# lucasgattas/ComfyUI-Egregora-Audio-Super-Resolution

Measured on AMD Instinct MI355X. Metric: audio-sec/sec (xRT) FlashSR 48kHz + Fat-Llama 800-iter at 1/2/4/8 MI355X, higher is better.
Workload: dtype f32(f16x2); 1 GPU; chain60: per GPU 60 s stereo 48 kHz; FlashSR (5.12 s chunks, hop 4.62 s, student_ldm 1-step + VAE + sr_vocoder, declared architecture, synthetic weights, chunk-sharded with one all-gather, WOLA) then Fat-Llama max_iterations=800 thr=0.6 normalize on autoscale off, threshold reading of the HEADLINE value: 'default' (SPEC.md section 3 default = absolute level on int16-scale samples, hard threshold, ; arch=gfx950:sramecc+:xnack-, chunks=13, rows_per_pass=32

## Files before the change

### comfyui-egregora-audio-super-resolution_amd/csrc/egr_nn_ops.hip

```cpp
#include <math.h>
#include <string.h>

#include <vector>

#include <stdlib.h>
#include <string.h>

#include "egr_common.h"
#include "egr_rowmax.h"
#include "egr_stft_tables.h"
#include "egr_plan.h"

namespace egr {

__global__ __launch_bounds__(256) void k_gn_stats(const float* __restrict__ x, int HW, int C, int G,
                                                   double* __restrict__ stats , int slab) {
    const int b = blockIdx.y;
    const int p0 = blockIdx.x * slab;
    const int p1 = min(HW, p0 + slab);
    const int cpg = C / G;
    const float* xb = x + (size_t)b * HW * C;
    for (int c = threadIdx.x; c < C; c += blockDim.x) {
        float s = 0.f, ss = 0.f;
        for (int p = p0; p < p1; ++p) {
// ... 261 lines not shown
        if (r0 + k < R && c0 + tx < Cc) t[k][tx] = x[off + (size_t)(r0 + k) * Cc + c0 + tx];
    __syncthreads();
    for (int k = ty; k < 32; k += 8)
        if (c0 + k < Cc && r0 + tx < R) y[off + (size_t)(c0 + k) * R + r0 + tx] = t[tx][k];
}

__global__ __launch_bounds__(256) void k_snake_aa(const float* __restrict__ x, const float* __restrict__ alpha,
                                                   const float* __restrict__ beta, const float* __restrict__ filt,
                                                   float* __restrict__ y, int L, int C, int K) {
    __shared__ float f[32];
    if (threadIdx.x < K) f[threadIdx.x] = filt[threadIdx.x];
    __syncthreads();
    const int b = blockIdx.z;
    const int c = blockIdx.x * 64 + (threadIdx.x & 63);
    const int l = blockIdx.y * 4 + (threadIdx.x >> 6);
    if (c >= C || l >= L) return;
    const float* xb = x + (size_t)b * L * C + c;
    const float a = __expf(alpha[c]), ib = 1.0f / (__expf(beta[c]) + 1e-9f);
    const int pad = K / 2 - 1;
    const int pl = pad * 2 + (K - 2) / 2;
    const int L2 = 2 * L;
    float acc = 0.f;
    for (int k = 0; k < K; ++k) {
        int i = 2 * l + k - (K / 2 - 1);
        i = i < 0 ? 0 : (i > L2 - 1 ? L2 - 1 : i);
        const int t = i + pl;
        int n_lo = (t - (K - 1) + 1) >> 1;
        if (2 * n_lo < t - (K - 1)) ++n_lo;
        const int n_hi = t >> 1;
        float u = 0.f;
        for (int n = n_lo; n <= n_hi; ++n) {
            int src = n - pad;
            src = src < 0 ? 0 : (src > L - 1 ? L - 1 : src);
            u += xb[(size_t)src * C] * f[t - 2 * n];
        }
        u *= 2.0f;
        const float sn = __sinf(u * a);
        acc += f[k] * (u + ib * sn * sn);
    }
    y[(size_t)b * L * C + (size_t)l * C + c] = acc;
}


template <int CB, int TL>
__global__ __launch_bounds__(256) void k_snake_aa_tiled(const float* __restrict__ x, const float* __restrict__ alpha,
                                                        const float* __restrict__ beta, const float* __restrict__ filt,
                                                        float* __restrict__ y, int L, int C) {
    constexpr int PL = 256 / CB, K = 12, XT = TL + 10, ST = 2 * TL + 10;
    __shared__ float xs[XT][CB];
    __shared__ float ss[ST][CB];
    __shared__ float f[K];
    if (threadIdx.x < K) f[threadIdx.x] = filt[threadIdx.x];
    const int c = threadIdx.x % CB, pl = threadIdx.x / CB;
    const int c0 = blockIdx.x * CB, l0 = blockIdx.y * TL, b = blockIdx.z;
    const float* xb = x + (size_t)b * L * C + c0 + c;
    for (int p = pl; p < XT; p += PL) {
        int src = l0 - 5 + p;
        src = src < 0 ? 0 : (src > L - 1 ? L - 1 : src);
        xs[p][c] = xb[(size_t)src * C];
    }
    const float a = __expf(alpha[c0 + c]), ib = 1.0f / (__expf(beta[c0 + c]) + 1e-9f);
    __syncthreads();
    const int L2 = 2 * L;
    for (int q = pl; q < ST; q += PL) {
        int i = 2 * l0 - 5 + q;
        i = i < 0 ? 0 : (i > L2 - 1 ? L2 - 1 : i);
        const int t = i + 15;
        const int n_hi = t >> 1;
        float u = 0.f;
#pragma unroll
        for (int j = 0; j < 6; ++j) {
            const int n = n_hi - j;
            int p = n - l0;
            p = p < 0 ? 0 : (p > XT - 1 ? XT - 1 : p);
            u += xs[p][c] * f[t - 2 * n];
        }
        u *= 2.0f;
        const float sn = __sinf(u * a);
        ss[q][c] = u + ib * sn * sn;
    }
    __syncthreads();
    float* yb = y + (size_t)b * L * C + c0 + c;
    for (int j = pl; j < TL; j += PL) {
        const int l = l0 + j;
        if (l >= L) break;
        float acc = 0.f;
#pragma unroll
        for (int k = 0; k < K; ++k) acc += f[k] * ss[2 * j + k][c];
        yb[(size_t)l * C] = acc;
    }
}

template <int J>
__global__ __launch_bounds__(256) void k_snake_aa_reg(const float* __restrict__ x, const float* __restrict__ alpha,
                                                      const float* __restrict__ beta, const float* __restrict__ filt,
                                                      float* __restrict__ y, int L, int C, int nruns,
                                                      unsigned* __restrict__ row_amax) {
    const int b = blockIdx.y;
    const long long per_row = (long long)nruns * C;
    float ymax = 0.f;
    for (long long gid = (long long)blockIdx.x * 256 + threadIdx.x; gid < per_row; gid += (long long)gridDim.x * 256) {
    const int c = (int)(gid % C);
    const int run = (int)(gid / C);
    const int l0 = run * J;
    float f[12];
#pragma unroll
    for (int k = 0; k < 12; ++k) f[k] = filt[k];
    const float a = __expf(alpha[c]), ib = 1.0f / (__expf(beta[c]) + 1e-9f);
    const float* xb = x + (size_t)b * L * C + c;
    float* yb = y + (size_t)b * L * C + c;
    const int L2 = 2 * L;
    float xw[J + 10];
#pragma unroll
    for (int i = 0; i < J + 10; ++i) {
        int src = l0 - 5 + i;
        src = src < 0 ? 0 : (src > L - 1 ? L - 1 : src);
        xw[i] = xb[(size_t)src * C];
    }
    float sv[2 * J + 10];
#pragma unroll
    for (int q = 0; q < 2 * J + 10; ++q) {
        float u = 0.f;
#pragma unroll
        for (int j = 0; j < 6; ++j) u += xw[5 + (q >> 1) - j] * f[(q & 1) + 2 * j];
        u *= 2.0f;
        const float sn = __sinf(u * a);
        sv[q] = u + ib * sn * sn;
    }
    const int i0 = 2 * l0 - 5;
    if (i0 < 0 || i0 + 2 * J + 9 > L2 - 1) {
        float s_first = 0.f, s_last = 0.f;
#pragma unroll
        for (int q = 0; q < 2 * J + 10; ++q) {
            if (i0 + q == 0) s_first = sv[q];
            if (i0 + q == L2 - 1) s_last = sv[q];
        }
#pragma unroll
        for (int q = 0; q < 2 * J + 10; ++q) {
            if (i0 + q < 0) sv[q] = s_first;
            if (i0 + q > L2 - 1) sv[q] = s_last;
        }
    }
#pragma unroll
    for (int jj = 0; jj < J; ++jj) {
        float acc = 0.f;
#pragma unroll
        for (int k = 0; k < 12; ++k) acc += f[k] * sv[2 * jj + k];
        if (l0 + jj < L) { yb[(size_t)(l0 + jj) * C] = acc; ymax = fmaxf(ymax, fabsf(acc)); }
    }
    }
    if (row_amax) row_amax_commit_wg(row_amax + (size_t)b * EGR_ROW_AMAX_STRIDE, ymax);
}

__global__ __launch_bounds__(256) void k_col2im1d(const float* __restrict__ Y, const float* __restrict__ bias,
                                                   const float* __restrict__ add, float* __restrict__ out, int Lin,
                                                   int Lout, int Co, int K, int r, int pad, long long n) {
    for (long long i = (long long)blockIdx.x * blockDim.x + threadIdx.x; i < n;
         i += (long long)gridDim.x * blockDim.x) {
        const int co = (int)(i % Co);
        const long long t = i / Co;
        const int o = (int)(t % Lout);
        const long long b = t / Lout;
        float v = bias ? bias[co] : 0.f;
        if (add) v += add[i];
        const int q = o + pad;
        for (int k = q % r; k < K; k += r) {
            const int ii = (q - k) / r;
            if (q - k >= 0 && ii < Lin) v += Y[(((size_t)b * Lin + ii) * K + k) * Co + co];
        }
        out[i] = v;
    }
}

__global__ __launch_bounds__(256) void k_stft_frames(const float* __restrict__ x, int L, int n_fft, int hop, int rpad,
                                                      int T, int t_valid, int ldm, const float* __restrict__ window,
                                                      FftDesc fd, const cplx* __restrict__ tw,
                                                      const cplx* __restrict__ wsplit, float* __restrict__ mag) {
    extern __shared__ __attribute__((aligned(16))) char smem[];
    const int Mh = n_fft / 2;
    cplx* cur = (cplx*)smem;
    cplx* alt = cur + Mh;
    const int t = blockIdx.x, b = blockIdx.y;
    float* o = mag + ((size_t)b * T + t) * ldm;
    if (t >= t_valid) {
        for (int k = threadIdx.x; k < ldm; k += blockDim.x) o[k] = 0.f;
        return;
    }
    const float* xb = x + (size_t)b * L;
    const int s0 = t * hop - rpad;
    for (int e = threadIdx.x; e < Mh; e += blockDim.x) {
        float v[2];
#pragma unroll
        for (int h = 0; h < 2; ++h) {
            int i = s0 + 2 * e + h;
            if (i < 0) i = -i;
            if (i > L - 1) i = 2 * (L - 1) - i;
            i = i < 0 ? 0 : (i > L - 1 ? L - 1 : i);
            v[h] = xb[i] * window[2 * e + h];
        }
        cur[e] = make_float2(v[0], v[1]);
    }
    __syncthreads();
    lds_fft<false>(cur, alt, fd, tw, 1, 0, 1, Mh, false);
    for (int k = threadIdx.x; k < ldm; k += blockDim.x) {
        float r = 0.f;
        if (k <= Mh) {
            const cplx Za = cur[k == Mh ? 0 : k];
            const cplx Zb = cur[(k == 0 || k == Mh) ? 0 : Mh - k];
            const cplx E = make_float2(0.5f * (Za.x + Zb.x), 0.5f * (Za.y - Zb.y));
            const cplx O = make_float2(0.5f * (Za.y + Zb.y), -0.5f * (Za.x - Zb.x));
            const cplx X = cadd(E, cmul(wsplit[k], O));
            r = sqrtf(X.x * X.x + X.y * X.y);
        }
        o[k] = r;
    }
}

__device__ __forceinline__ void philox_round(unsigned& c0, unsigned& c1, unsigned& c2, unsigned& c3, unsigned k0,
                                             unsigned k1) {
    const unsigned long long p0 = (unsigned long long)0xD2511F53u * c0;
    const unsigned long long p1 = (unsigned long long)0xCD9E8D57u * c2;
    const unsigned n0 = (unsigned)(p1 >> 32) ^ c1 ^ k0, n1 = (unsigned)p1;
    const unsigned n2 = (unsigned)(p0 >> 32) ^ c3 ^ k1, n3 = (unsigned)p0;
    c0 = n0; c1 = n1; c2 = n2; c3 = n3;
}

__global__ __launch_bounds__(256) void k_randn(float* __restrict__ out, long long per_row, int rows,
                                                unsigned long long seed, const long long* __restrict__ row_ids, long long id_base) {
    const long long quads = (per_row + 3) / 4;
    const long long n = quads * rows;
    for (long long i = (long long)blockIdx.x * blockDim.x + threadIdx.x; i < n;
         i += (long long)gridDim.x * blockDim.x) {
        const int r = (int)(i / quads);
        const long long q = i - (long long)r * quads;
        const unsigned long long rid = row_ids ? (unsigned long long)row_ids[r] : (unsigned long long)(id_base + r);
        unsigned c0 = (unsigned)q, c1 = (unsigned)(q >> 32), c2 = (unsigned)rid, c3 = (unsigned)(rid >> 32);
        unsigned k0 = (unsigned)seed, k1 = (unsigned)(seed >> 32);
#pragma unroll
        for (int it = 0; it < 10; ++it) {
            philox_round(c0, c1, c2, c3, k0, k1);
            k0 += 0x9E3779B9u;
            k1 += 0xBB67AE85u;
        }
        const float u0 = ((float)c0 + 0.5f) * 2.3283064365386963e-10f, u1 = ((float)c1 + 0.5f) * 2.3283064365386963e-10f;
        const float u2 = ((float)c2 + 0.5f) * 2.3283064365386963e-10f, u3 = ((float)c3 + 0.5f) * 2.3283064365386963e-10f;
        const float r0 = sqrtf(-2.0f * logf(u0)), r1 = sqrtf(-2.0f * logf(u2));
        float z[4];
        z[0] = r0 * cosf(6.283185307179586f * u1);
        z[1] = r0 * sinf(6.283185307179586f * u1);
        z[2] = r1 * cosf(6.283185307179586f * u3);
        z[3] = r1 * sinf(6.283185307179586f * u3);
        float* o = out + (size_t)r * per_row + q * 4;
        for (int j = 0; j < 4; ++j)
            if (q * 4 + j < per_row) o[j] = z[j];
    }
}

__global__ __launch_bounds__(256) void k_wino_in(const float* __restrict__ x, int B, int H, int W, int C, int TH, int TW,
                                                  const float* __restrict__ gsc, const float* __restrict__ gsh, int gsilu,
                                                  float* __restrict__ V) {
    const int C4 = C >> 2;
    const long long P = (long long)B * TH * TW, total = P * C4;
    for (long long i = (long long)blockIdx.x * blockDim.x + threadIdx.x; i < total; i += (long long)gridDim.x * blockDim.x) {
        const int c4 = (int)(i % C4);
        const long long t = i / C4;
        const int tx = (int)(t % TW), ty = (int)((t / TW) % TH), b = (int)(t / ((long long)TW * TH));
        float4 d[4][4];
        float4 sc = make_float4(1.f, 1.f, 1.f, 1.f), sh = make_float4(0.f, 0.f, 0.f, 0.f);
        if (gsc) {
            sc = *(const float4*)(gsc + (size_t)b * C + 4 * c4);
            sh = *(const float4*)(gsh + (size_t)b * C + 4 * c4);
        }
#pragma unroll
        for (int r = 0; r < 4; ++r) {
            const int iy = 2 * ty - 1 + r;
#pragma unroll
            for (int q = 0; q < 4; ++q) {
                const int ix = 2 * tx - 1 + q;
                const bool ok = (unsigned)iy < (unsigned)H && (unsigned)ix < (unsigned)W;
                const size_t off = ok ? (((size_t)b * H + iy) * W + ix) * C + 4 * c4 : (size_t)(4 * c4);
                float4 v = *(const float4*)(x + off);
                if (gsc) {
                    v = make_float4(v.x * sc.x + sh.x, v.y * sc.y + sh.y, v.z * sc.z + sh.z, v.w * sc.w + sh.w);
                    if (gsilu) {
                        v.x = v.x / (1.f + __expf(-v.x)); v.y = v.y / (1.f + __expf(-v.y));
                        v.z = v.z / (1.f + __expf(-v.z)); v.w = v.w / (1.f + __expf(-v.w));
                    }
                }
                d[r][q] = ok ? v : make_float4(0.f, 0.f, 0.f, 0.f);
            }
        }
#define F4OP(a, op, b) make_float4(a.x op b.x, a.y op b.y, a.z op b.z, a.w op b.w)
        float4 r_[4][4];
#pragma unroll
        for (int q = 0; q < 4; ++q) {
            r_[0][q] = F4OP(d[0][q], -, d[2][q]);
            r_[1][q] = F4OP(d[1][q], +, d[2][q]);
            r_[2][q] = F4OP(d[2][q], -, d[1][q]);
            r_[3][q] = F4OP(d[1][q], -, d[3][q]);
        }
        float* o = V + (size_t)t * C + 4 * c4;
        const size_t zs = (size_t)P * C;
#pragma unroll
        for (int r = 0; r < 4; ++r) {
            *(float4*)(o + (size_t)(4 * r + 0) * zs) = F4OP(r_[r][0], -, r_[r][2]);
            *(float4*)(o + (size_t)(4 * r + 1) * zs) = F4OP(r_[r][1], +, r_[r][2]);
// ... 213 lines not shown
extern "C" int egr_groupnorm_coeff_from_stats(const double* stats, const float* gamma, const float* beta, int B, int HW, int C,
                                              int G, float eps, float* scale, float* shift, void* stream) {
    EGR_CHECK(stats && gamma && beta && scale && shift && B >= 1 && HW >= 1 && C >= 1 && G >= 1 && C % G == 0, EGR_ERR_ARG,
              "bad argument");
    hipLaunchKernelGGL(k_gn_coeff, dim3((B * C + 255) / 256), dim3(256), 0, (hipStream_t)stream, stats, gamma, beta, scale, shift,
                       B, C, G, (double)HW * (C / G), eps);
    EGR_HIP(hipGetLastError());
    return EGR_OK;
}

extern "C" int egr_gn_operand_bound(const float* scale, const float* shift, int B, int C, const float* x_row_amax, float* bound, void* stream) {
    EGR_CHECK(scale && shift && x_row_amax && bound && B >= 1 && C >= 1, EGR_ERR_ARG, "bad argument");
    hipLaunchKernelGGL(k_gn_bound, dim3(B), dim3(256), 0, (hipStream_t)stream, scale, shift, C, x_row_amax, bound);
    EGR_HIP(hipGetLastError());
    return EGR_OK;
}

extern "C" size_t egr_groupnorm_workspace_bytes(int B, int C, int G) {
    return sizeof(double) * (size_t)B * G * 2 + sizeof(float) * 2 * (size_t)B * C + 64;
}

extern "C" int egr_layernorm_rows_ra(const float* x, const float* gamma, const float* beta, float* y, int64_t rows, int C,
                                     float eps, int batch_rows, float* row_amax, void* stream) {
    EGR_CHECK(x && gamma && beta && y && rows >= 1 && C >= 1 && batch_rows >= 1 && batch_rows <= 65535 && rows % batch_rows == 0, EGR_ERR_ARG,
              "bad argument");
    const long long per_b = rows / batch_rows;
    long long nx = (per_b + 3) / 4, cap = std::max<long long>(1, 16384 / batch_rows);
    if (nx > cap) nx = cap;
    hipLaunchKernelGGL(k_layernorm, dim3((unsigned)nx, (unsigned)batch_rows), dim3(256), 0, (hipStream_t)stream, x, gamma, beta, y,
                       (int)per_b, C, eps, (unsigned*)row_amax);
    EGR_HIP(hipGetLastError());
    return EGR_OK;
}

extern "C" int egr_layernorm_rows(const float* x, const float* gamma, const float* beta, float* y, int64_t rows, int C,
                                  float eps, void* stream) {
    int g = 1;
    for (int c : {64, 32, 16, 8, 4, 2}) if (rows % c == 0) { g = c; break; }
    return egr_layernorm_rows_ra(x, gamma, beta, y, rows, C, eps, g, nullptr, stream);
}

extern "C" int egr_softmax_rows(float* x, int64_t rows, int cols, void* stream) {
    EGR_CHECK(x && rows >= 1 && cols >= 1, EGR_ERR_ARG, "bad argument");
    const dim3 grid((unsigned)rows), blk(256);
    if (cols <= 1024) hipLaunchKernelGGL(k_softmax_reg<4>, grid, blk, 0, (hipStream_t)stream, x, cols);
    else if (cols <= 2048) hipLaunchKernelGGL(k_softmax_reg<8>, grid, blk, 0, (hipStream_t)stream, x, cols);
    else if (cols <= 4096) hipLaunchKernelGGL(k_softmax_reg<16>, grid, blk, 0, (hipStream_t)stream, x, cols);
    else hipLaunchKernelGGL(k_softmax, grid, blk, 0, (hipStream_t)stream, x, cols);
    EGR_HIP(hipGetLastError());
    return EGR_OK;
}

extern "C" int egr_eltwise_ra(const float* a, const float* b, float* y, int64_t n, int op, float s0, float s1, int batch_rows,
                              float* row_amax, void* stream) {
    EGR_CHECK(a && y && n >= 0 && op >= 0 && op <= 5 && batch_rows >= 1 && batch_rows <= 65535 && n % batch_rows == 0, EGR_ERR_ARG, "bad argument");
    EGR_CHECK(b || (op != EW_ADD && op != EW_AXPBY && op != EW_ADD_SCALE), EGR_ERR_ARG, "binary op needs b");
    if (n == 0) return EGR_OK;
    const long long per = n / batch_rows;
    hipLaunchKernelGGL(k_eltwise, dim3(row_grid_x(per, batch_rows, 8192, 4), (unsigned)batch_rows), dim3(256), 0, (hipStream_t)stream, a, b, y, per,
                       op, s0, s1, (unsigned*)row_amax);
    EGR_HIP(hipGetLastError());
    return EGR_OK;
}

extern "C" int egr_eltwise(const float* a, const float* b, float* y, int64_t n, int op, float s0, float s1, void* stream) {
    int g = 1;
    for (int c : {64, 32, 16, 8, 4, 2}) if (n % c == 0) { g = c; break; }
    return egr_eltwise_ra(a, b, y, n, op, s0, s1, g, nullptr, stream);
}

extern "C" int egr_geglu_ra(const float* u, float* y, int64_t rows, int D, int batch_rows, float* row_amax, void* stream) {
    EGR_CHECK(u && y && rows >= 1 && D >= 1 && batch_rows >= 1 && batch_rows <= 65535 && rows % batch_rows == 0, EGR_ERR_ARG, "bad argument");
    const long long per = rows / batch_rows;
    hipLaunchKernelGGL(k_geglu, dim3(row_grid_x(per * D, batch_rows, 8192, 4), (unsigned)batch_rows), dim3(256), 0, (hipStream_t)stream, u, y, per, D,
                       (unsigned*)row_amax);
    EGR_HIP(hipGetLastError());
    return EGR_OK;
}

extern "C" int egr_geglu(const float* u, float* y, int64_t rows, int D, void* stream) {
    int g = 1;
    for (int c : {64, 32, 16, 8, 4, 2}) if (rows % c == 0) { g = c; break; }
    return egr_geglu_ra(u, y, rows, D, g, nullptr, stream);
}

extern "C" int egr_tap_gather(const float* P, const float* bias, float* y, int B, int H, int W, int KH, int KW, int Cout, int pad_t,
                              int pad_l, void* stream) {
    EGR_CHECK(P && y && B >= 1 && H >= 1 && W >= 1 && KH >= 1 && KW >= 1 && Cout >= 1, EGR_ERR_ARG, "bad argument");
    hipLaunchKernelGGL(k_tap_gather, dim3(grid1d((long long)B * H * W * Cout)), dim3(256), 0, (hipStream_t)stream, P, bias, y, B, H, W,
                       KH, KW, Cout, pad_t, pad_l);
    EGR_HIP(hipGetLastError());
    return EGR_OK;
}

extern "C" int egr_conv_cin1(const float* x, const float* w_packed, const float* bias, float* y, int B, int H, int W, int Cout, int KH,
                             int KW, int pad_t, int pad_l, void* stream) {
    EGR_CHECK(x && w_packed && y && B >= 1 && H >= 1 && W >= 1 && Cout >= 4 && Cout % 4 == 0 && 256 % (Cout / 4) == 0, EGR_ERR_ARG,
              "bad argument (Cout / 4 must divide 256)");
    EGR_CHECK((KH == 3 && KW == 3) || (KH == 1 && KW == 1), EGR_ERR_UNSUPPORTED, "one-input-channel conv: 3x3 or 1x1 only");
    EGR_CHECK((long long)B * H * W < (1ll << 31), EGR_ERR_ARG, "image too large for 32-bit pixel indices");
    EGR_CHECK((((uintptr_t)y) & 15) == 0 && (!bias || (((uintptr_t)bias) & 15) == 0), EGR_ERR_ARG, "y / bias need 16-byte alignment");
    const int ppi = 256 / (Cout / 4);
    long long nb = ((long long)B * H * W + ppi - 1) / ppi;
    if (nb > 8192) nb = 8192;
    if (KH == 3) hipLaunchKernelGGL((k_conv_cin1<9>), dim3((unsigned)nb), dim3(256), 0, (hipStream_t)stream, x, w_packed, bias, y, B, H, W,
                                    Cout, KW, pad_t, pad_l);
    else hipLaunchKernelGGL((k_conv_cin1<1>), dim3((unsigned)nb), dim3(256), 0, (hipStream_t)stream, x, w_packed, bias, y, B, H, W, Cout,
                            KW, pad_t, pad_l);
    EGR_HIP(hipGetLastError());
    return EGR_OK;
}

extern "C" int egr_concat_channels_ra(const float* a, const float* b, float* y, int64_t M, int C1, int C2, int batch_rows, float* row_amax,
                                      void* stream) {
    EGR_CHECK(a && b && y && M >= 1 && C1 >= 1 && C2 >= 1 && batch_rows >= 1 && batch_rows <= 65535 && M % batch_rows == 0, EGR_ERR_ARG, "bad argument");
    const long long per = M / batch_rows;
    hipLaunchKernelGGL(k_concat, dim3(row_grid_x(per * (C1 + C2), batch_rows, 8192, 4), (unsigned)batch_rows), dim3(256), 0, (hipStream_t)stream, a, b, y,
                       per, C1, C2, (unsigned*)row_amax);
    EGR_HIP(hipGetLastError());
    return EGR_OK;
}

extern "C" int egr_concat_channels(const float* a, const float* b, float* y, int64_t M, int C1, int C2, void* stream) {
    int g = 1;
    for (int c : {64, 32, 16, 8, 4, 2}) if (M % c == 0) { g = c; break; }
    return egr_concat_channels_ra(a, b, y, M, C1, C2, g, nullptr, stream);
}

extern "C" int egr_transpose_batched(const float* x, float* y, int batch, int R, int Cc, void* stream) {
    EGR_CHECK(x && y && batch >= 1 && batch <= 65535 && R >= 1 && Cc >= 1, EGR_ERR_ARG, "bad argument");
    hipLaunchKernelGGL(k_transpose, dim3((Cc + 31) / 32, (R + 31) / 32, batch), dim3(256), 0, (hipStream_t)stream, x, y, R,
                       Cc);
    EGR_HIP(hipGetLastError());
    return EGR_OK;
}

extern "C" int egr_snake_aa_ra(const float* x, const float* alpha, const float* beta, const float* filt, float* y, int B,
                               int L, int C, int K, float* row_amax, void* stream);
extern "C" int egr_snake_aa(const float* x, const float* alpha, const float* beta, const float* filt, float* y, int B,
                            int L, int C, int K, void* stream) {
    return egr_snake_aa_ra(x, alpha, beta, filt, y, B, L, C, K, nullptr, stream);
}

extern "C" int egr_snake_aa_ra(const float* x, const float* alpha, const float* beta, const float* filt, float* y, int B,
                               int L, int C, int K, float* row_amax, void* stream) {
    EGR_CHECK(x && alpha && beta && filt && y && B >= 1 && B <= 65535 && L >= 1 && C >= 1 && K >= 2 && K <= 32 && K % 2 == 0,
              EGR_ERR_ARG, "bad argument");
    hipStream_t st = (hipStream_t)stream;
    static const bool tiled = getenv("EGR_SNAKE") && !strcmp(getenv("EGR_SNAKE"), "tiled");
    if (K == 12 && !tiled) {
        constexpr int J = 16;
        const int nruns = (L + J - 1) / J;
        static const int max_wg = getenv("EGR_SNAKE_WG") ? atoi(getenv("EGR_SNAKE_WG")) : 8192;
        hipLaunchKernelGGL((k_snake_aa_reg<J>), dim3(row_grid_x((long long)nruns * C, B, max_wg), (unsigned)B), dim3(256), 0, st, x, alpha, beta, filt, y, L, C,
                           nruns, (unsigned*)row_amax);
        row_amax = nullptr;
    } else if (K == 12 && C % 64 == 0)
        hipLaunchKernelGGL((k_snake_aa_tiled<64, 32>), dim3(C / 64, (L + 31) / 32, B), dim3(256), 0, st, x, alpha, beta, filt, y, L, C);
    else if (K == 12 && C % 32 == 0)
        hipLaunchKernelGGL((k_snake_aa_tiled<32, 64>), dim3(C / 32, (L + 63) / 64, B), dim3(256), 0, st, x, alpha, beta, filt, y, L, C);
    else if (K == 12 && C % 16 == 0)
        hipLaunchKernelGGL((k_snake_aa_tiled<16, 128>), dim3(C / 16, (L + 127) / 128, B), dim3(256), 0, st, x, alpha, beta, filt, y, L, C);
    else
        hipLaunchKernelGGL(k_snake_aa, dim3((C + 63) / 64, (L + 3) / 4, B), dim3(256), 0, st, x, alpha, beta, filt, y, L, C, K);
    EGR_HIP(hipGetLastError());
    if (row_amax) return egr_absmax_rows(y, B, (int64_t)L * C, 1, 0, row_amax, stream);
    return EGR_OK;
}

extern "C" int egr_col2im_convtr1d(const float* Y, const float* bias, const float* add, float* out, int B, int Lin,
                                   int Lout, int Co, int K, int r, int pad, void* stream) {
    EGR_CHECK(Y && out && B >= 1 && Lin >= 1 && Lout >= 1 && Co >= 1 && K >= 1 && r >= 1 && pad >= 0, EGR_ERR_ARG,
              "bad argument");
    const long long n = (long long)B * Lout * Co;
    hipLaunchKernelGGL(k_col2im1d, dim3(grid1d(n)), dim3(256), 0, (hipStream_t)stream, Y, bias, add, out, Lin, Lout, Co, K,
                       r, pad, n);
    EGR_HIP(hipGetLastError());
    return EGR_OK;
}

extern "C" int egr_stft_frames(const float* x, int B, int L, int n_fft, int hop, int rpad, int T, int t_valid, int ldm,
                               const float* window, float* mag, void* stream) {
    EGR_CHECK(x && window && mag && B >= 1 && B <= 65535 && L >= 2 && hop >= 1 && T >= 1 && t_valid >= 0 && t_valid <= T,
              EGR_ERR_ARG, "bad argument");
    EGR_CHECK(n_fft >= 4 && n_fft % 2 == 0 && n_fft <= 8192 && ldm >= n_fft / 2 + 1 && rpad < L, EGR_ERR_UNSUPPORTED,
              "bad STFT geometry");
    StftTables t;
    int rc = stft_tables(n_fft, &t);
    if (rc) return rc;
    const size_t lds = (size_t)2 * (n_fft / 2) * sizeof(float2);
    hipLaunchKernelGGL(k_stft_frames, dim3(T, B), dim3(256), lds, (hipStream_t)stream, x, L, n_fft, hop, rpad, T, t_valid,
                       ldm, window, t.fd, t.tw, t.wsplit, mag);
    EGR_HIP(hipGetLastError());
    return EGR_OK;
}

extern "C" int egr_randn_base(float* out, int64_t per_row, int rows, uint64_t seed, const int64_t* row_ids, int64_t id_base, void* stream) {
    EGR_CHECK(out && per_row >= 1 && rows >= 1, EGR_ERR_ARG, "bad argument");
    const long long n = ((per_row + 3) / 4) * rows;
    hipLaunchKernelGGL(k_randn, dim3(grid1d(n)), dim3(256), 0, (hipStream_t)stream, out, (long long)per_row, rows,
                       (unsigned long long)seed, (const long long*)row_ids, (long long)id_base);
    EGR_HIP(hipGetLastError());
    return EGR_OK;
}

extern "C" int egr_randn(float* out, int64_t per_row, int rows, uint64_t seed, const int64_t* row_ids, void* stream) {
    return egr_randn_base(out, per_row, rows, seed, row_ids, 0, stream);
}

extern "C" int egr_lowpass_gain(const float* mag, int B, int T, int ldm, int nb, float pct, float sr, int order,
                                float ripple_db, int64_t nbins, int* cut_out, float* gain, void* stream) {
    EGR_CHECK(mag && cut_out && gain && B >= 1 && B <= 65535 && T >= 1 && nb >= 2 && nb <= ldm && nbins >= 2 && order >= 1,
              EGR_ERR_ARG, "bad argument");
    hipStream_t st = (hipStream_t)stream;
    hipLaunchKernelGGL(k_cutoff_bin, dim3(B), dim3(256), nb * sizeof(float), st, mag, T, ldm, nb, pct, cut_out);
    const float eps2 = powf(10.0f, ripple_db / 10.0f) - 1.0f;
    hipLaunchKernelGGL(k_cheby_gain, dim3(grid1d(nbins), B), dim3(256), 0, st, cut_out, nb, sr, order, eps2, (long long)nbins,
                       gain);
    EGR_HIP(hipGetLastError());
    return EGR_OK;
}

extern "C" int egr_winograd_input(const float* x, const float* gn_scale, const float* gn_shift, int gn_silu, int B, int H,
                                  int W, int C, float* V, void* stream) {
    EGR_CHECK(x && V && B >= 1 && H >= 1 && W >= 1 && C >= 4 && C % 4 == 0 && (!gn_scale || gn_shift), EGR_ERR_ARG,
              "bad argument");
    const int TH = (H + 1) / 2, TW = (W + 1) / 2;
    const long long n = (long long)B * TH * TW * (C / 4);
    hipLaunchKernelGGL(k_wino_in, dim3(grid1d(n)), dim3(256), 0, (hipStream_t)stream, x, B, H, W, C, TH, TW, gn_scale,
                       gn_shift, gn_silu, V);
    EGR_HIP(hipGetLastError());
    return EGR_OK;
}

extern "C" int egr_winograd_output(const float* M, const float* bias, const float* res, float* y, int B, int H, int W, int N,
                                   int act, void* stream) {
    EGR_CHECK(M && y && B >= 1 && H >= 1 && W >= 1 && N >= 4 && N % 4 == 0 && (act == 0 || act == 1), EGR_ERR_ARG,
              "bad argument");
    const int TH = (H + 1) / 2, TW = (W + 1) / 2;
    const long long n = (long long)B * TH * TW * (N / 4);
    hipLaunchKernelGGL(k_wino_out, dim3(grid1d(n)), dim3(256), 0, (hipStream_t)stream, M, bias, res, B, H, W, N, TH, TW, act, y);
    EGR_HIP(hipGetLastError());
    return EGR_OK;
}
```

### comfyui-egregora-audio-super-resolution_amd/csrc/egr_nn_wino4.hip

```cpp
#include "egr_common.h"
#include "egr_rowmax.h"

namespace egr {

#define W4_A 0.75
#define W4_B 1.5
static constexpr float kA = (float)W4_A, kB = (float)W4_B, kA2 = kA * kA, kB2 = kB * kB, kA3 = kA2 * kA, kB3 = kB2 * kB;
static constexpr float kC0 = kA2 * kB2, kC2 = -(kA2 + kB2);

#define F4A(a, b) make_float4(a.x + b.x, a.y + b.y, a.z + b.z, a.w + b.w)
#define F4S(a, b) make_float4(a.x - b.x, a.y - b.y, a.z - b.z, a.w - b.w)
#define F4M(s, a) make_float4((s) * a.x, (s) * a.y, (s) * a.z, (s) * a.w)
#define F4FMA(s, a, b) make_float4(fmaf((s), a.x, b.x), fmaf((s), a.y, b.y), fmaf((s), a.z, b.z), fmaf((s), a.w, b.w))

#ifdef EGR_W4_NT
typedef float f4v __attribute__((ext_vector_type(4)));
__device__ __forceinline__ void st_f4(float* p, const float4& v) {
    f4v t = {v.x, v.y, v.z, v.w};
    __builtin_nontemporal_store(t, (f4v*)p);
}
#else
__device__ __forceinline__ void st_f4(float* p, const float4& v) { *(float4*)p = v; }
#endif

__device__ __forceinline__ void bt6(const float4 (&d)[6], float4 (&t)[6]) {
    const float4 ea = F4FMA(-kB2, d[2], d[4]);
    const float4 oa = F4M(kA, F4FMA(-kB2, d[1], d[3]));
    const float4 eb = F4FMA(-kA2, d[2], d[4]);
    const float4 ob = F4M(kB, F4FMA(-kA2, d[1], d[3]));
    t[0] = F4FMA(kC0, d[0], F4FMA(kC2, d[2], d[4]));
    t[1] = F4A(ea, oa);
    t[2] = F4S(ea, oa);
    t[3] = F4A(eb, ob);
    t[4] = F4S(eb, ob);
    t[5] = F4FMA(kC0, d[1], F4FMA(kC2, d[3], d[5]));
}

__device__ __forceinline__ void at6(const float4 (&m)[6], float4 (&s)[4]) {
    const float4 pa = F4A(m[1], m[2]), ma = F4S(m[1], m[2]), pb = F4A(m[3], m[4]), mb = F4S(m[3], m[4]);
    s[0] = F4A(F4A(m[0], pa), pb);
    s[1] = F4FMA(kA, ma, F4M(kB, mb));
    s[2] = F4FMA(kA2, pa, F4M(kB2, pb));
    s[3] = F4A(F4FMA(kA3, ma, F4M(kB3, mb)), m[5]);
}

template <bool GN, bool SILU>
__global__ __launch_bounds__(256) void k_wino4_in(const float* __restrict__ x, int B, int H, int W, int C, int TH, int TW,
                                                   const float* __restrict__ gsc, const float* __restrict__ gsh,
                                                   float* __restrict__ V, unsigned* __restrict__ row_amax) {
    const int C4 = C >> 2;
    const long long P = (long long)B * TH * TW;
    const size_t zs = (size_t)P * C;
    const int b = blockIdx.y;
    const long long per_img = (long long)TH * TW * C4;
    float vmax = 0.f;
    for (long long ii = (long long)blockIdx.x * blockDim.x + threadIdx.x; ii < per_img; ii += (long long)gridDim.x * blockDim.x) {
        {
        const int c4 = (int)(ii % C4);
        const int tl = (int)(ii / C4);
        const int tx = tl % TW, ty = tl / TW;
        const long long t = (long long)b * TH * TW + tl;
        float4 d[6][6];
#pragma unroll
        for (int r = 0; r < 6; ++r) {
            const int iy = 4 * ty - 1 + r;
#pragma unroll
            for (int q = 0; q < 6; ++q) {
                const int ix = 4 * tx - 1 + q;
                const bool ok = (unsigned)iy < (unsigned)H && (unsigned)ix < (unsigned)W;
                const size_t off = ok ? (((size_t)b * H + iy) * W + ix) * C + 4 * c4 : (size_t)(4 * c4);
                d[r][q] = *(const float4*)(x + off);
            }
        }
        const bool interior = ty > 0 && tx > 0 && 4 * ty + 4 < H && 4 * tx + 4 < W;
        if (GN) {
            const float4 sc = *(const float4*)(gsc + (size_t)b * C + 4 * c4);
            const float4 sh = *(const float4*)(gsh + (size_t)b * C + 4 * c4);
#pragma unroll
            for (int r = 0; r < 6; ++r)
#pragma unroll
                for (int q = 0; q < 6; ++q) {
                    float4 v = d[r][q];
                    v = make_float4(v.x * sc.x + sh.x, v.y * sc.y + sh.y, v.z * sc.z + sh.z, v.w * sc.w + sh.w);
                    if (SILU) {
                        v.x = v.x / (1.f + __expf(-v.x)); v.y = v.y / (1.f + __expf(-v.y));
                        v.z = v.z / (1.f + __expf(-v.z)); v.w = v.w / (1.f + __expf(-v.w));
                    }
                    d[r][q] = v;
                }
        }
        if (!interior) {
#pragma unroll
            for (int r = 0; r < 6; ++r) {
                const int iy = 4 * ty - 1 + r;
#pragma unroll
                for (int q = 0; q < 6; ++q) {
                    const int ix = 4 * tx - 1 + q;
                    if (!((unsigned)iy < (unsigned)H && (unsigned)ix < (unsigned)W)) d[r][q] = make_float4(0.f, 0.f, 0.f, 0.f);
                }
            }
        }
#pragma unroll
        for (int q = 0; q < 6; ++q) {
            float4 col[6], o6[6];
#pragma unroll
            for (int r = 0; r < 6; ++r) col[r] = d[r][q];
            bt6(col, o6);
#pragma unroll
            for (int r = 0; r < 6; ++r) d[r][q] = o6[r];
        }
        float* o = V + (size_t)t * C + 4 * c4;
#pragma unroll
        for (int r = 0; r < 6; ++r) {
            float4 row[6];
            bt6(d[r], row);
#pragma unroll
            for (int q = 0; q < 6; ++q) {
                st_f4(o + (size_t)(6 * r + q) * zs, row[q]);
                vmax = amax4(row[q], vmax);
            }
        }
        }
    }
    if (row_amax) row_amax_commit(row_amax + (size_t)b * EGR_ROW_AMAX_STRIDE, vmax);
}

template <bool RES, bool SILU, bool STATS>
__global__ __launch_bounds__(256) void k_wino4_out(const float* __restrict__ Mx, const float* __restrict__ bias,
                                                    const float* __restrict__ res, int B, int H, int W, int N, int TH, int TW,
                                                    float* __restrict__ y, float2* __restrict__ part, unsigned* __restrict__ row_amax) {
    const int N4 = N >> 2;
    const long long P = (long long)B * TH * TW;
    const size_t zs = (size_t)P * N;
    const int b = blockIdx.y;
    const long long per_img = (long long)TH * TW * N4;
    float ymax = 0.f;
    for (long long ii = (long long)blockIdx.x * blockDim.x + threadIdx.x; ii < per_img; ii += (long long)gridDim.x * blockDim.x) {
        {
        const int n4 = (int)(ii % N4);
        const int tl = (int)(ii / N4);
        const int tx = tl % TW, ty = tl / TW;
        const long long t = (long long)b * TH * TW + tl;
        const long long i = t * N4 + n4;
        const float* mi = Mx + (size_t)t * N + 4 * n4;
        float4 s[4][6];
#pragma unroll
        for (int q = 0; q < 6; ++q) {
            float4 m[6];
#pragma unroll
            for (int r = 0; r < 6; ++r) m[r] = *(const float4*)(mi + (size_t)(6 * r + q) * zs);
            float4 col[4];
            at6(m, col);
#pragma unroll
            for (int a = 0; a < 4; ++a) s[a][q] = col[a];
        }
        float4 bv = make_float4(0.f, 0.f, 0.f, 0.f);
        if (bias) bv = *(const float4*)(bias + 4 * n4);
        float ps = 0.f, pq = 0.f;
#pragma unroll
        for (int a = 0; a < 4; ++a) {
            const size_t off = (((size_t)b * H + 4 * ty + a) * W + 4 * tx) * N + 4 * n4;
            float4 rr[4];
            if (RES) {
#pragma unroll
                for (int c = 0; c < 4; ++c) rr[c] = *(const float4*)(res + off + (size_t)c * N);
            }
            float4 o[4];
            at6(s[a], o);
#pragma unroll
            for (int c = 0; c < 4; ++c) {
                float4 v = F4A(o[c], bv);
                if (RES) v = F4A(v, rr[c]);
                if (SILU) {
                    v.x = v.x / (1.f + __expf(-v.x)); v.y = v.y / (1.f + __expf(-v.y));
                    v.z = v.z / (1.f + __expf(-v.z)); v.w = v.w / (1.f + __expf(-v.w));
                }
                *(float4*)(y + off + (size_t)c * N) = v;
                ymax = amax4(v, ymax);
                if (STATS) {
                    ps += (v.x + v.y) + (v.z + v.w);
                    pq += (v.x * v.x + v.y * v.y) + (v.z * v.z + v.w * v.w);
                }
            }
        }
        if (STATS) part[i] = make_float2(ps, pq);
        }
    }
    if (row_amax) row_amax_commit(row_amax + (size_t)b * EGR_ROW_AMAX_STRIDE, ymax);
}

__global__ __launch_bounds__(256) void k_gn_from_partials(const float2* __restrict__ part, int tiles_per_image, int N4, int q4,
                                                           double* __restrict__ stats) {
    __shared__ double rs[256], rq[256];
    const int g = blockIdx.x, b = blockIdx.y, G = gridDim.x;
    const float2* pb = part + (size_t)b * tiles_per_image * N4 + (size_t)g * q4;
    double s = 0.0, q = 0.0;
    const long long n = (long long)tiles_per_image * q4;
    for (long long e = threadIdx.x; e < n; e += 256) {
        const long long t = e / q4;
        const int j = (int)(e - t * q4);
        const float2 v = pb[t * N4 + j];
        s += (double)v.x;
        q += (double)v.y;
    }
    rs[threadIdx.x] = s;
    rq[threadIdx.x] = q;
    __syncthreads();
    for (int o = 128; o > 0; o >>= 1) {
        if (threadIdx.x < o) { rs[threadIdx.x] += rs[threadIdx.x + o]; rq[threadIdx.x] += rq[threadIdx.x + o]; }
        __syncthreads();
    }
    if (threadIdx.x == 0) {
        stats[((size_t)b * G + g) * 2 + 0] = rs[0];
        stats[((size_t)b * G + g) * 2 + 1] = rq[0];
    }
}

static inline int grid1d(long long n) {
    long long b = (n + 255) / 256;
    return (int)(b < 1 ? 1 : (b > 16384 ? 16384 : b));
}

}

using namespace egr;

extern "C" int egr_winograd4_g(double* g18) {
    EGR_CHECK(g18, EGR_ERR_ARG, "null g18");
    const double a = W4_A, b = W4_B, n0 = a * a * b * b, na = 2 * a * a * (a * a - b * b), nb = 2 * b * b * (b * b - a * a);
    const double pts[5] = {0.0, a, -a, b, -b}, nn[5] = {n0, na, na, nb, nb};
    for (int j = 0; j < 5; ++j) {
        g18[3 * j + 0] = 1.0 / nn[j];
        g18[3 * j + 1] = pts[j] / nn[j];
        g18[3 * j + 2] = pts[j] * pts[j] / nn[j];
    }
    g18[15] = 0.0; g18[16] = 0.0; g18[17] = 1.0;
    return EGR_OK;
}

extern "C" int egr_winograd4_input_ra(const float* x, const float* gn_scale, const float* gn_shift, int gn_silu, int B, int H,
                                      int W, int C, float* V, float* row_amax, void* stream);
extern "C" int egr_winograd4_input(const float* x, const float* gn_scale, const float* gn_shift, int gn_silu, int B, int H,
                                   int W, int C, float* V, void* stream) {
    return egr_winograd4_input_ra(x, gn_scale, gn_shift, gn_silu, B, H, W, C, V, nullptr, stream);
}

extern "C" int egr_winograd4_input_ra(const float* x, const float* gn_scale, const float* gn_shift, int gn_silu, int B, int H,
                                      int W, int C, float* V, float* row_amax, void* stream) {
    EGR_CHECK(x && V && B >= 1 && H >= 4 && W >= 4 && H % 4 == 0 && W % 4 == 0 && C >= 4 && C % 4 == 0 &&
                  (!gn_scale || gn_shift), EGR_ERR_ARG, "F(4x4,3x3) input transform needs H, W, C multiples of 4");
    const int TH = H / 4, TW = W / 4;
    EGR_CHECK(B <= 65535, EGR_ERR_ARG, "too many images");
    const dim3 g(row_grid_x((long long)TH * TW * (C / 4), B), (unsigned)B), blk(256);
    hipStream_t st = (hipStream_t)stream;
    unsigned* ra = (unsigned*)row_amax;
    if (!gn_scale) hipLaunchKernelGGL((k_wino4_in<false, false>), g, blk, 0, st, x, B, H, W, C, TH, TW, gn_scale, gn_shift, V, ra);
    else if (gn_silu) hipLaunchKernelGGL((k_wino4_in<true, true>), g, blk, 0, st, x, B, H, W, C, TH, TW, gn_scale, gn_shift, V, ra);
    else hipLaunchKernelGGL((k_wino4_in<true, false>), g, blk, 0, st, x, B, H, W, C, TH, TW, gn_scale, gn_shift, V, ra);
    EGR_HIP(hipGetLastError());
    return EGR_OK;
}

static int wino4_out_launch(const float* M, const float* bias, const float* res, float* y, int B, int H, int W, int N, int act,
                            float2* part, unsigned* row_amax, hipStream_t st) {
    const int TH = H / 4, TW = W / 4;
    EGR_CHECK(B <= 65535, EGR_ERR_ARG, "too many images");
    const dim3 g(row_grid_x((long long)TH * TW * (N / 4), B), (unsigned)B), blk(256);
#define W4O(R_, S_, T_) hipLaunchKernelGGL((k_wino4_out<R_, S_, T_>), g, blk, 0, st, M, bias, res, B, H, W, N, TH, TW, y, part, row_amax)
    if (part) {
        if (res && act) W4O(true, true, true); else if (res) W4O(true, false, true);
        else if (act) W4O(false, true, true); else W4O(false, false, true);
    } else {
        if (res && act) W4O(true, true, false); else if (res) W4O(true, false, false);
        else if (act) W4O(false, true, false); else W4O(false, false, false);
    }
#undef W4O
    EGR_HIP(hipGetLastError());
    return EGR_OK;
}

extern "C" int egr_winograd4_output(const float* M, const float* bias, const float* res, float* y, int B, int H, int W, int N,
                                    int act, void* stream) {
    EGR_CHECK(M && y && B >= 1 && H >= 4 && W >= 4 && H % 4 == 0 && W % 4 == 0 && N >= 4 && N % 4 == 0 &&
                  (act == 0 || act == 1), EGR_ERR_ARG, "F(4x4,3x3) output transform needs H, W, N multiples of 4");
    return wino4_out_launch(M, bias, res, y, B, H, W, N, act, nullptr, nullptr, (hipStream_t)stream);
}

extern "C" int egr_winograd4_output_stats(const float* M, const float* bias, const float* res, float* y, int B, int H, int W,
                                          int N, int act, void* part, void* stream) {
    EGR_CHECK(M && y && part && B >= 1 && H >= 4 && W >= 4 && H % 4 == 0 && W % 4 == 0 && N >= 4 && N % 4 == 0 &&
                  (act == 0 || act == 1), EGR_ERR_ARG, "F(4x4,3x3) output transform needs H, W, N multiples of 4");
    return wino4_out_launch(M, bias, res, y, B, H, W, N, act, (float2*)part, nullptr, (hipStream_t)stream);
}

extern "C" int egr_winograd4_output_ra(const float* M, const float* bias, const float* res, float* y, int B, int H, int W, int N,
                                       int act, void* part, float* row_amax, void* stream) {
    EGR_CHECK(M && y && B >= 1 && H >= 4 && W >= 4 && H % 4 == 0 && W % 4 == 0 && N >= 4 && N % 4 == 0 &&
                  (act == 0 || act == 1), EGR_ERR_ARG, "F(4x4,3x3) output transform needs H, W, N multiples of 4");
    return wino4_out_launch(M, bias, res, y, B, H, W, N, act, (float2*)part, (unsigned*)row_amax, (hipStream_t)stream);
}

extern "C" int egr_groupnorm_stats_from_partials(const void* part, int B, int tiles_per_image, int C, int G, double* stats,
                                                 void* stream) {
    EGR_CHECK(part && stats && B >= 1 && B <= 65535 && tiles_per_image >= 1 && C >= 4 && G >= 1 && C % G == 0 && (C / G) % 4 == 0,
              EGR_ERR_ARG, "bad argument");
    hipLaunchKernelGGL(k_gn_from_partials, dim3(G, B), dim3(256), 0, (hipStream_t)stream, (const float2*)part, tiles_per_image, C / 4,
                       (C / G) / 4, stats);
    EGR_HIP(hipGetLastError());
    return EGR_OK;
}
```

Baseline: 279.0 audio-sec/sec.

## Add span-based snake AA kernel and banded Winograd-4 input transform with halo reuse

Adds a snake anti-alias kernel in which each thread walks a span of consecutive runs and carries the 10-sample input and upsampled halo forward, so overlapping halo loads and sin evaluations are not recomputed per run. Adds a banded Winograd F(4x4,3x3) input transform in which each thread processes a vertical band of tiles and reuses the two overlapping rows through shared memory, with XCD-aware chunk assignment. Both paths are on by default and can be switched off with environment variables. The trade-off is less parallelism per launch and higher register/LDS pressure, and the heuristics could pick poor span or band sizes for some shapes.

```diff
diff --git a/comfyui-egregora-audio-super-resolution_amd/csrc/egr_nn_ops.hip b/comfyui-egregora-audio-super-resolution_amd/csrc/egr_nn_ops.hip
--- a/comfyui-egregora-audio-super-resolution_amd/csrc/egr_nn_ops.hip
+++ b/comfyui-egregora-audio-super-resolution_amd/csrc/egr_nn_ops.hip
@@ -437,6 +437,88 @@
     if (row_amax) row_amax_commit_wg(row_amax + (size_t)b * EGR_ROW_AMAX_STRIDE, ymax);
 }
 
+template <int J>
+__global__ __launch_bounds__(256) void k_snake_aa_span(const float* __restrict__ x, const float* __restrict__ alpha,
+                                                       const float* __restrict__ beta, const float* __restrict__ filt,
+                                                       float* __restrict__ y, int L, int C, int nruns, int S, int nspans,
+                                                       unsigned* __restrict__ row_amax) {
+    const int b = blockIdx.y;
+    const long long per_row = (long long)nspans * C;
+    float ymax = 0.f;
+    for (long long gid = (long long)blockIdx.x * 256 + threadIdx.x; gid < per_row; gid += (long long)gridDim.x * 256) {
+    const int c = (int)(gid % C);
+    const int span = (int)(gid / C);
+    const int r0 = span * S, r1 = r0 + S < nruns ? r0 + S : nruns;
+    float f[12];
+#pragma unroll
+    for (int k = 0; k < 12; ++k) f[k] = filt[k];
+    const float a = __expf(alpha[c]), ib = 1.0f / (__expf(beta[c]) + 1e-9f);
+    const float* xb = x + (size_t)b * L * C + c;
+    float* yb = y + (size_t)b * L * C + c;
+    const int L2 = 2 * L;
+    float xw[J + 10];
+    float sv[2 * J + 10];
+#pragma unroll
+    for (int i = 0; i < 10; ++i) {
+        int src = r0 * J - 5 + i;
+        src = src < 0 ? 0 : (src > L - 1 ? L - 1 : src);
+        xw[i] = xb[(size_t)src * C];
+    }
+#pragma unroll
+    for (int q = 0; q < 10; ++q) {
+        float u = 0.f;
+#pragma unroll
+        for (int j = 0; j < 6; ++j) u += xw[5 + (q >> 1) - j] * f[(q & 1) + 2 * j];
+        u *= 2.0f;
+        const float sn = __sinf(u * a);
+        sv[q] = u + ib * sn * sn;
+    }
+#pragma unroll 1
+    for (int run = r0; run < r1; ++run) {
+    const int l0 = run * J;
+#pragma unroll
+    for (int i = 10; i < J + 10; ++i) {
+        int src = l0 - 5 + i;
+        src = src < 0 ? 0 : (src > L - 1 ? L - 1 : src);
+        xw[i] = xb[(size_t)src * C];
+    }
+#pragma unroll
+    for (int q = 10; q < 2 * J + 10; ++q) {
+        float u = 0.f;
+#pragma unroll
+        for (int j = 0; j < 6; ++j) u += xw[5 + (q >> 1) - j] * f[(q & 1) + 2 * j];
+        u *= 2.0f;
+        const float sn = __sinf(u * a);
+        sv[q] = u + ib * sn * sn;
+    }
+    const int i0 = 2 * l0 - 5;
+    if (i0 < 0 || i0 + 2 * J + 9 > L2 - 1) {
+        float s_first = 0.f, s_last = 0.f;
+#pragma unroll
+        for (int q = 0; q < 2 * J + 10; ++q) {
+            if (i0 + q == 0) s_first = sv[q];
+            if (i0 + q == L2 - 1) s_last = sv[q];
+        }
+#pragma unroll
+        for (int q = 0; q < 2 * J + 10; ++q) {
+            if (i0 + q < 0) sv[q] = s_first;
+            if (i0 + q > L2 - 1) sv[q] = s_last;
+        }
+    }
+#pragma unroll
+    for (int jj = 0; jj < J; ++jj) {
+        float acc = 0.f;
+#pragma unroll
+        for (int k = 0; k < 12; ++k) acc += f[k] * sv[2 * jj + k];
+        if (l0 + jj < L) { yb[(size_t)(l0 + jj) * C] = acc; ymax = fmaxf(ymax, fabsf(acc)); }
+    }
+#pragma unroll
+    for (int i = 0; i < 10; ++i) { xw[i] = xw[J + i]; sv[i] = sv[2 * J + i]; }
+    }
+    }
+    if (row_amax) row_amax_commit_wg(row_amax + (size_t)b * EGR_ROW_AMAX_STRIDE, ymax);
+}
+
 __global__ __launch_bounds__(256) void k_col2im1d(const float* __restrict__ Y, const float* __restrict__ bias,
                                                    const float* __restrict__ add, float* __restrict__ out, int Lin,
                                                    int Lout, int Co, int K, int r, int pad, long long n) {
@@ -956,6 +1038,14 @@
         constexpr int J = 16;
         const int nruns = (L + J - 1) / J;
         static const int max_wg = getenv("EGR_SNAKE_WG") ? atoi(getenv("EGR_SNAKE_WG")) : 8192;
+        static const int span_env = getenv("EGR_SNAKE_SPAN") ? atoi(getenv("EGR_SNAKE_SPAN")) : -1;
+        if (span_env != 0) {
+            int S = span_env > 0 ? span_env : 8;
+            if (span_env < 0) while (S > 1 && (long long)((nruns + S - 1) / S) * C * B < 256LL * 1024) S >>= 1;
+            const int nspans = (nruns + S - 1) / S;
+            hipLaunchKernelGGL((k_snake_aa_span<J>), dim3(row_grid_x((long long)nspans * C, B, max_wg), (unsigned)B), dim3(256), 0, st, x, alpha, beta, filt, y,
+                               L, C, nruns, S, nspans, (unsigned*)row_amax);
+        } else
         hipLaunchKernelGGL((k_snake_aa_reg<J>), dim3(row_grid_x((long long)nruns * C, B, max_wg), (unsigned)B), dim3(256), 0, st, x, alpha, beta, filt, y, L, C,
                            nruns, (unsigned*)row_amax);
         row_amax = nullptr;
diff --git a/comfyui-egregora-audio-super-resolution_amd/csrc/egr_nn_wino4.hip b/comfyui-egregora-audio-super-resolution_amd/csrc/egr_nn_wino4.hip
--- a/comfyui-egregora-audio-super-resolution_amd/csrc/egr_nn_wino4.hip
+++ b/comfyui-egregora-audio-super-resolution_amd/csrc/egr_nn_wino4.hip
@@ -120,6 +120,118 @@
                 vmax = amax4(row[q], vmax);
             }
         }
+        }
+    }
+    if (row_amax) row_amax_commit(row_amax + (size_t)b * EGR_ROW_AMAX_STRIDE, vmax);
+}
+
+template <bool GN, bool SILU, bool FIRST>
+__device__ __forceinline__ void wino4_in_tile(const float* __restrict__ xb, int H, int W, int C, int tx, int ty, const unsigned (&co)[6],
+                                              const float4& sc, const float4& sh, float4* __restrict__ cy, float* __restrict__ V,
+                                              unsigned o, size_t zs, float& vmax) {
+    constexpr int R0 = FIRST ? 0 : 2;
+    float4 d[6][6];
+#pragma unroll
+    for (int r = R0; r < 6; ++r) {
+        int iy = 4 * ty - 1 + r;
+        iy = iy < 0 ? 0 : (iy > H - 1 ? H - 1 : iy);
+        const unsigned ro = (unsigned)iy * (unsigned)W * (unsigned)C;
+#pragma unroll
+        for (int q = 0; q < 6; ++q) d[r][q] = *(const float4*)(xb + (ro + co[q]));
+    }
+    const bool interior = ty > 0 && tx > 0 && 4 * ty + 4 < H && 4 * tx + 4 < W;
+    if (GN) {
+#pragma unroll
+        for (int r = R0; r < 6; ++r)
+#pragma unroll
+            for (int q = 0; q < 6; ++q) {
+                float4 v = d[r][q];
+                v = make_float4(v.x * sc.x + sh.x, v.y * sc.y + sh.y, v.z * sc.z + sh.z, v.w * sc.w + sh.w);
+                if (SILU) {
+                    v.x = v.x / (1.f + __expf(-v.x)); v.y = v.y / (1.f + __expf(-v.y));
+                    v.z = v.z / (1.f + __expf(-v.z)); v.w = v.w / (1.f + __expf(-v.w));
+                }
+                d[r][q] = v;
+            }
+    }
+    if (!interior) {
+#pragma unroll
+        for (int r = R0; r < 6; ++r) {
+            const int iy = 4 * ty - 1 + r;
+#pragma unroll
+            for (int q = 0; q < 6; ++q) {
+                const int ix = 4 * tx - 1 + q;
+                if (!((unsigned)iy < (unsigned)H && (unsigned)ix < (unsigned)W)) d[r][q] = make_float4(0.f, 0.f, 0.f, 0.f);
+            }
+        }
+    }
+#pragma unroll
+    for (int q = 0; q < 6; ++q) {
+        if (!FIRST) { d[0][q] = cy[256 * q]; d[1][q] = cy[256 * (6 + q)]; }
+        cy[256 * q] = d[4][q];
+        cy[256 * (6 + q)] = d[5][q];
+    }
+#pragma unroll
+    for (int q = 0; q < 6; ++q) {
+        float4 col[6], o6[6];
+#pragma unroll
+        for (int r = 0; r < 6; ++r) col[r] = d[r][q];
+        bt6(col, o6);
+#pragma unroll
+        for (int r = 0; r < 6; ++r) d[r][q] = o6[r];
+    }
+#pragma unroll
+    for (int r = 0; r < 6; ++r) {
+        float4 row[6];
+        bt6(d[r], row);
+#pragma unroll
+        for (int q = 0; q < 6; ++q) {
+            st_f4(V + (size_t)(6 * r + q) * zs + o, row[q]);
+            vmax = amax4(row[q], vmax);
+        }
+    }
+}
+
+template <bool GN, bool SILU>
+__global__ __launch_bounds__(256) void k_wino4_in_band(const float* __restrict__ x, int B, int H, int W, int C, int TH, int TW,
+                                                        const float* __restrict__ gsc, const float* __restrict__ gsh,
+                                                        float* __restrict__ V, unsigned* __restrict__ row_amax, int lq, int lx,
+                                                        int bh, int nbx, int nby, int nchunks) {
+    __shared__ float4 carry[12 * 256];
+    const int C4 = C >> 2;
+    const size_t zs = (size_t)B * TH * TW * C;
+    const int b = blockIdx.y;
+    const float* xb = x + (size_t)b * H * W * C;
+    float* Vb = V + (size_t)b * TH * TW * C;
+    const int cq = threadIdx.x & ((1 << lq) - 1), txl = (threadIdx.x >> lq) & ((1 << lx) - 1), tyl = threadIdx.x >> (lq + lx);
+    const int ly = 8 - lq - lx;
+    const int per_xcd = (nchunks + 7) >> 3, wg_per_xcd = gridDim.x >> 3;
+    float vmax = 0.f;
+    for (int k = blockIdx.x >> 3; k < per_xcd; k += wg_per_xcd) {
+        const int chunk = (blockIdx.x & 7) * per_xcd + k;
+        if (chunk >= nchunks) break;
+        const int by = chunk % nby, bx = (chunk / nby) % nbx, sl = chunk / (nby * nbx);
+        const int c4 = (sl << lq) + cq, tx = (bx << lx) + txl, ty0 = ((by << ly) + tyl) * bh;
+        if (c4 >= C4 || tx >= TW || ty0 >= TH) continue;
+        const int ty1 = ty0 + bh < TH ? ty0 + bh : TH;
+        float4 sc = make_float4(0.f, 0.f, 0.f, 0.f), sh = sc;
+        if (GN) {
+            sc = *(const float4*)(gsc + (size_t)b * C + 4 * c4);
+            sh = *(const float4*)(gsh + (size_t)b * C + 4 * c4);
+        }
+        unsigned co[6];
+#pragma unroll
+        for (int q = 0; q < 6; ++q) {
+            int ix = 4 * tx - 1 + q;
+            ix = ix < 0 ? 0 : (ix > W - 1 ? W - 1 : ix);
+            co[q] = (unsigned)ix * (unsigned)C + 4u * (unsigned)c4;
+        }
+        unsigned o = ((unsigned)ty0 * (unsigned)TW + (unsigned)tx) * (unsigned)C + 4u * (unsigned)c4;
+        wino4_in_tile<GN, SILU, true>(xb, H, W, C, tx, ty0, co, sc, sh, carry + threadIdx.x, Vb, o, zs, vmax);
+#pragma unroll 1
+        for (int ty = ty0 + 1; ty < ty1; ++ty) {
+            o += (unsigned)TW * (unsigned)C;
+            wino4_in_tile<GN, SILU, false>(xb, H, W, C, tx, ty, co, sc, sh, carry + threadIdx.x, Vb, o, zs, vmax);
         }
     }
     if (row_amax) row_amax_commit(row_amax + (size_t)b * EGR_ROW_AMAX_STRIDE, vmax);
@@ -251,9 +363,36 @@
                   (!gn_scale || gn_shift), EGR_ERR_ARG, "F(4x4,3x3) input transform needs H, W, C multiples of 4");
     const int TH = H / 4, TW = W / 4;
     EGR_CHECK(B <= 65535, EGR_ERR_ARG, "too many images");
-    const dim3 g(row_grid_x((long long)TH * TW * (C / 4), B), (unsigned)B), blk(256);
+    const dim3 blk(256);
     hipStream_t st = (hipStream_t)stream;
     unsigned* ra = (unsigned*)row_amax;
+    static const int band_env = getenv("EGR_W4_BAND") ? atoi(getenv("EGR_W4_BAND")) : -1;
+    if (band_env != 0 && (long long)H * W * C < (1LL << 30)) {
+        const int C4 = C / 4;
+        int lq = 0, lx = 0;
+        while (lq < 4 && (1 << lq) < C4) ++lq;
+        while (lx < 4 && (1 << lx) < TW) ++lx;
+        while (lq + lx < 8 && (1 << lq) < C4) ++lq;
+        while (lq + lx < 8 && (1 << lx) < TW) ++lx;
+        const int ly = 8 - lq - lx;
+        const int nsl = (C4 + (1 << lq) - 1) >> lq, nbx = (TW + (1 << lx) - 1) >> lx;
+        int bh = band_env > 0 ? band_env : 8;
+        auto chunks_at = [&](int h) { return (long long)nsl * nbx * (((TH + h - 1) / h + (1 << ly) - 1) >> ly); };
+        if (band_env < 0) while (bh > 1 && chunks_at(bh) * B < 768) bh >>= 1;
+        const int nby = ((TH + bh - 1) / bh + (1 << ly) - 1) >> ly;
+        const long long nchunks = chunks_at(bh);
+        EGR_CHECK(nchunks < (1LL << 30), EGR_ERR_ARG, "tensor too large");
+        long long gx = (nchunks + 7) & ~7LL, cap = (4096 / B) & ~7;
+        if (cap < 8) cap = 8;
+        if (gx > cap) gx = cap;
+        const dim3 g((unsigned)gx, (unsigned)B);
+#define W4I(G_, S_) hipLaunchKernelGGL((k_wino4_in_band<G_, S_>), g, blk, 0, st, x, B, H, W, C, TH, TW, gn_scale, gn_shift, V, ra, lq, lx, bh, nbx, nby, (int)nchunks)
+        if (!gn_scale) W4I(false, false); else if (gn_silu) W4I(true, true); else W4I(true, false);
+#undef W4I
+        EGR_HIP(hipGetLastError());
+        return EGR_OK;
+    }
+    const dim3 g(row_grid_x((long long)TH * TW * (C / 4), B), (unsigned)B);
     if (!gn_scale) hipLaunchKernelGGL((k_wino4_in<false, false>), g, blk, 0, st, x, B, H, W, C, TH, TW, gn_scale, gn_shift, V, ra);
     else if (gn_silu) hipLaunchKernelGGL((k_wino4_in<true, true>), g, blk, 0, st, x, B, H, W, C, TH, TW, gn_scale, gn_shift, V, ra);
     else hipLaunchKernelGGL((k_wino4_in<true, false>), g, blk, 0, st, x, B, H, W, C, TH, TW, gn_scale, gn_shift, V, ra);
```

Measured after the change: 282.6 audio-sec/sec, median of 6. 1.3% higher.
